# maniacs-oss/shadow

Measured on AMD Instinct MI355X. Metric: routing-table build GTEPS + packet-routes/sec at 1/2/4/8 MI355X (%HBM roofline), higher is better.
Workload: dtype f64

## Files before the change

### shadow_amd/csrc/topo_sssp_batch.hip

```cpp
#include <hip/hip_runtime.h>
#include <hipcub/hipcub.hpp>

#include <algorithm>
#include <cmath>
#include <cstddef>
#include <cstdint>
#include <type_traits>

#include "topo_dev_common.h"

namespace shdtopo {

namespace {

using namespace dev;

constexpr int kBatchRB = 2;
constexpr int kBatchU = 2;
constexpr int kBChunk = 512;
#ifndef SHD_BATCH_WRCOUNT
#define SHD_BATCH_WRCOUNT 0
#endif
#ifndef SHD_BATCH_TIME
#define SHD_BATCH_TIME 0
// ... 186 lines not shown
template <int K>
__device__ __forceinline__ double h0_bound(const LdsB<K>& L, const BView<K>& D, uint32_t j) {
    return fmin(L.hs[j], bits2d(D.get(0u, j)));
}

struct BBuckets {
    double inv_delta;
    uint32_t cb;
    uint32_t tie_tag;
};

constexpr uint32_t kTagMask = 0x3FFFFFFFu;
constexpr uint32_t kTagClaim = 0x40000000u;
static_assert(kTagMask == kPairTagMask && kTagClaim == kPairTagClaim, "the pair walks' tag (topo_device.h)");
constexpr uint32_t kTagTie = 0x80000000u;
__device__ __forceinline__ bool tag_claimed(uint32_t w, uint32_t ep) {
    return (w & ~kTagTie) == (ep | kTagClaim);
}
__device__ __forceinline__ bool tag_tied(uint32_t w, uint32_t ep) {
    return (w & kTagTie) && (w & kTagMask) == ep;
}

__device__ __forceinline__ uint32_t kappa_cut(const DevCSR& g, float4 ks0, float4 ks1, double T,
                                              uint32_t r0, uint32_t deg) {
    if ((double)ks0.x > T) return 0;
    if ((double)ks0.y > T) return 1;
    if ((double)ks0.z > T) return 3;
    if ((double)ks0.w > T) return 7;
    if (kKProbes > 4) {
        if ((double)ks1.x > T) return 15;
        if ((double)ks1.y > T) return 31;
        if ((double)ks1.z > T) return 63;
        if ((double)ks1.w > T) return 127;
    }
    uint32_t lo = kKProbes > 4 ? 128u : 8u, hi = deg;
    while (lo < hi) {
        const uint32_t mid = (lo + hi) >> 1;
        if ((double)g.kap[r0 + mid] > T) hi = mid; else lo = mid + 1;
    }
    return lo;
}

template <int K, bool CUT = false, bool DIR = false>
__device__ __forceinline__ uint32_t load_chunk(const uint32_t* Q, uint32_t cnt, const DevCSR& g,
                                               LdsB<K>& L, const BView<K>& D,
                                               typename MaskOps<K>::M* mcur,
                                               typename MaskOps<K>::M* hcur, bool stats = true,
                                               uint32_t spec_to = 0u) {
    using MO = MaskOps<K>;
    const uint32_t tid = threadIdx.x;
    const unsigned long long t0 = wall_clock64();
    uint32_t deg = 0;
    unsigned long long act = 0;
    if (tid < cnt) {
        const uint32_t v = Q[tid];
        uint32_t m;
        if (v < D.H) {
            m = MO::take(hcur, v);
            if (spec_to) {
                const uint32_t xw = D.xb[(v * K) >> 5] >> ((v * K) & 31);
                for (int jj = 0; jj < K; jj++) {
                    if (((m >> jj) & 1u) || ((xw >> jj) & 1u)) continue;
                    const unsigned long long d = D.hd[(size_t)v * K + jj];
                    if (d != kInfBits && bkt(bits2d(d), L.sh[jj], L.invd) <= spec_to) m |= 1u << jj;
                }
                if (m) atomicOr(&D.xb[(v * K) >> 5], m << ((v * K) & 31));
            }
        } else {
            wl_count(L, WL_MASK_ST, true, mcur + v);
            m = MO::take(mcur, v);
        }
        const uint32_t* rp = (CUT || !DIR) ? g.rowptr : g.rowptr_in;
        const uint32_t r0 = rp[v], r1 = rp[v + 1];
        deg = m ? r1 - r0 : 0u;
        if (CUT && deg) {
            const float4 ks0 = g.ksum[kKProbes / 4 * (size_t)v];
            const float4 ks1 = kKProbes > 4 ? g.ksum[kKProbes / 4 * (size_t)v + 1] : ks0;
            double dv[K];
            if (v < D.H) {
#pragma unroll
                for (int jj = 0; jj < K; jj++) dv[jj] = bits2d(D.hd[(size_t)v * K + jj]);
            } else {
                typedef unsigned long long u64x2 __attribute__((ext_vector_type(2)));
                const u64x2* p = reinterpret_cast<const u64x2*>(D.dist + (size_t)v * K);
#pragma unroll
                for (int h = 0; h < K / 2; h++) {
                    const u64x2 x = __builtin_nontemporal_load(p + h);
                    dv[2 * h] = bits2d(x.x);
                    dv[2 * h + 1] = bits2d(x.y);
                }
            }
            double T = -INFINITY;
#pragma unroll
            for (int jj = 0; jj < K; jj++) {
                if (!((m >> jj) & 1u)) continue;
                L.val[tid * K + jj] = dv[jj];
                const double h = h0_bound(L, D, (uint32_t)jj);
                const double t = (h - dv[jj]) + 1e-5 * (h + dv[jj] + g.piMax) + 1e-9;
                T = t > T ? t : T;
            }
            const uint32_t c = kappa_cut(g, ks0, ks1, T, r0, deg);
            deg = c < deg ? c : deg;
        }
        act = (unsigned long long)deg * (unsigned long long)__popc(m);
        L.rs[tid] = r0;
        L.vx[tid] = v;
        L.msk[tid] = m;
        if (stats && v < D.H && deg) {
            atomicAdd(&L.dg[0], (unsigned long long)deg);
            atomicAdd(&L.dg[1], act);
        }
    }
    uint32_t total;
    const uint32_t off = block_excl_scan<kSsspBlock>(deg, L.wave, &total);
    if (tid < cnt) L.off[tid] = off;
    if (tid == 0) L.off[cnt] = total;
    act = wave_sum_u64(act);
    if (stats && (tid & 63) == 0 && act) atomicAdd(&L.cnt[0], act);
    if (!CUT) {
        for (uint32_t i = tid; i < cnt * K; i += kSsspBlock) {
            const uint32_t vi = i / K, jj = i % K;
            if ((L.msk[vi] >> jj) & 1u) L.val[i] = bits2d(D.get(L.vx[vi], jj));
        }
    }
    if (tid < (uint32_t)K) L.dh0[tid] = h0_bound(L, D, tid);
    __syncthreads();
    if (stats && tid == 0) {
        L.cnt[2] += total;
        L.cnt[3] += wall_clock64() - t0;
    }
    return total;
}

__device__ __forceinline__ double rec_pi(uint32_t p) {
    if (kKapInRec) return (double)(float)__builtin_bit_cast(_Float16, (unsigned short)(p >> 16));
    return (double)__uint_as_float(p);
}
__device__ __forceinline__ float rec_kap0(uint32_t p) {
    return (float)__builtin_bit_cast(_Float16, (unsigned short)(p & 0xFFFFu));
}

__device__ __forceinline__ bool kappa_useful(float k0, double h, double d, double pimax) {
    return (double)k0 <= (h - d) + 1e-5 * (h + d + pimax) + 1e-9;
}

template <int K>
__device__ __forceinline__ int chunk_slot(const LdsB<K>& L, uint32_t cnt, uint32_t e) {
    int lo = 0, hi = (int)cnt - 1;
    while (lo < hi) {
        const int mid = (lo + hi + 1) >> 1;
        if (L.off[mid] <= e) lo = mid; else hi = mid - 1;
    }
    return lo;
}

__device__ __forceinline__ uint32_t wave_excl_scan(uint32_t x, uint32_t* total) {
    const uint32_t lane = threadIdx.x & 63;
    uint32_t v = x;
#pragma unroll
    for (int o = 1; o < 64; o <<= 1) {
        const uint32_t y = __shfl_up(v, o, 64);
        if (lane >= (uint32_t)o) v += y;
    }
    *total = __shfl(v, 63, 64);
    return v - x;
}

__device__ __forceinline__ uint32_t slice_slot(const uint32_t* off, uint32_t cnt, uint32_t e) {
    uint32_t lo = 0, hi = cnt - 1;
    while (lo < hi) {
        const uint32_t mid = (lo + hi + 1) >> 1;
        if (off[mid] <= e) lo = mid; else hi = mid - 1;
    }
    return lo;
}

constexpr uint32_t kBSub = kBChunk / (kSsspBlock / 64);
template <int K>
__device__ __forceinline__ uint32_t load_sub(uint32_t qv, uint32_t cnt, uint32_t wb,
                                             const DevCSR& g, LdsB<K>& L, const BView<K>& D,
                                             typename MaskOps<K>::M* mcur) {
    using MO = MaskOps<K>;
    const uint32_t lane = threadIdx.x & 63;
    uint32_t deg = 0;
    unsigned long long act = 0;
    if (lane < K) L.dh0[lane] = h0_bound(L, D, lane);
    if (lane < cnt) {
        const uint32_t v = qv;
        wl_count(L, WL_MASK_ST, true, mcur + v);
        const uint32_t m = MO::take(mcur, v);
        rl_count(L, RL_CHUNK, true, mcur + v);
        rl_count(L, RL_CHUNK, true, g.rowptr + v);
        rl_count(L, RL_CHUNK, true, g.ksum + kKProbes / 4 * (size_t)v);
        rl_count(L, RL_CHUNK, true, D.dist + (size_t)v * K);
        const uint32_t r0 = g.rowptr[v], r1 = g.rowptr[v + 1];
        const float4 ks0 = g.ksum[kKProbes / 4 * (size_t)v];
        const float4 ks1 = kKProbes > 4 ? g.ksum[kKProbes / 4 * (size_t)v + 1] : ks0;
        double dv[K];
        {
            typedef unsigned long long u64x2 __attribute__((ext_vector_type(2)));
            const u64x2* p = reinterpret_cast<const u64x2*>(D.dist + (size_t)v * K);
#pragma unroll
            for (int h = 0; h < K / 2; h++) {
                const u64x2 x = __builtin_nontemporal_load(p + h);
                dv[2 * h] = bits2d(x.x);
                dv[2 * h + 1] = bits2d(x.y);
            }
        }
        deg = m ? r1 - r0 : 0u;
        if (deg) {
            double T = -INFINITY;
#pragma unroll
            for (int jj = 0; jj < K; jj++) {
                if (!((m >> jj) & 1u)) continue;
                L.val[(wb + lane) * K + jj] = dv[jj];
                const double h = h0_bound(L, D, (uint32_t)jj);
                const double t = (h - dv[jj]) + 1e-5 * (h + dv[jj] + g.piMax) + 1e-9;
                T = t > T ? t : T;
            }
            const uint32_t c = kappa_cut(g, ks0, ks1, T, r0, deg);
            deg = c < deg ? c : deg;
        }
        act = (unsigned long long)deg * (unsigned long long)__popc(m);
        L.rs[wb + lane] = r0;
        L.vx[wb + lane] = v;
        L.msk[wb + lane] = m;
    }
    uint32_t total;
    const uint32_t off = wave_excl_scan(deg, &total);
    if (lane < cnt) L.off[wb + lane] = off;
    act = wave_sum_u64(act);
    if (lane == 0) {
        if (act) atomicAdd(&L.cnt[0], act);
        atomicAdd(&L.cnt[2], (unsigned long long)total);
    }
    asm volatile("s_waitcnt lgkmcnt(0)" ::: "memory");
    __builtin_amdgcn_wave_barrier();
    return total;
}

template <int K, int UA, bool WAVE = false>
__device__ __forceinline__ void relax_batch_t(const uint32_t* Q, uint32_t nq, const DevCSR& g,
                                              LdsB<K>& L, const BView<K>& D,
                                              typename MaskOps<K>::M* mcur,
                                              typename MaskOps<K>::M* hdef,
                                              typename MaskOps<K>::M* mnxt, uint32_t* qout,
                                              uint32_t qcap, uint32_t* hq, const BBuckets& B) {
    using MO = MaskOps<K>;
    static_assert(64 % K == 0, "a wave holds whole edge groups");
    static_assert(UA >= 1 && (UA & (UA - 1)) == 0, "the phase-B edge search halves UA * 64");
    constexpr int RB = kBatchRB;
    const uint32_t tid = threadIdx.x;
    const uint32_t lane = tid & 63;
    const uint32_t wv = tid >> 6;
    const uint32_t wb = WAVE ? wv * kBSub : 0u;
    uint32_t nb0 = 0, nqv = 0;
#if SHD_BATCH_TIME
    unsigned long long bt_last = wall_clock64();
#endif
    if (WAVE) {
        if (lane == 0) nb0 = atomicAdd(&L.qhead, kBSub);
        nb0 = __shfl(nb0, 0, 64);
        rl_count(L, RL_CHUNK, nb0 + lane < nq, Q + nb0 + lane);
        nqv = nb0 + lane < nq ? Q[nb0 + lane] : 0u;
    }
    for (uint32_t base = 0;; base += kBChunk) {
        uint32_t cnt, total;
        if (WAVE) {
            const uint32_t b0 = nb0, qv = nqv;
            if (b0 >= nq) break;
            cnt = min(kBSub, nq - b0);
            if (lane == 0) nb0 = atomicAdd(&L.qhead, kBSub);
            nb0 = __shfl(nb0, 0, 64);
            rl_count(L, RL_CHUNK, nb0 + lane < nq, Q + nb0 + lane);
            nqv = nb0 + lane < nq ? Q[nb0 + lane] : 0u;
            total = load_sub<K>(qv, cnt, wb, g, L, D, mcur);
        } else {
            if (base >= nq) break;
            cnt = min((uint32_t)kBChunk, nq - base);
            total = load_chunk<K, true>(Q + base, cnt, g, L, D, mcur, hdef, true,
                                        B.cb);
        }
        BT_TICK(0);
        constexpr uint32_t kStep = WAVE ? 64u : (uint32_t)kSsspBlock;
        for (uint32_t eb = 0; eb < total; eb += kStep * UA) {
            uint32_t an[UA], amk[UA], alo[UA], awl[UA], awh[UA], apb[UA];
#pragma unroll
            for (int a = 0; a < UA; a++) {
                const uint32_t e = eb + (uint32_t)a * kStep + (WAVE ? 0u : wv * 64) + lane;
                const bool valid = e < total;
                const int lo = !valid ? 0
                               : WAVE ? (int)(wb + slice_slot(L.off + wb, cnt, e))
                                      : chunk_slot<K>(L, cnt, e);
                const uint32_t jr = valid ? L.rs[lo] + (e - L.off[lo]) : 0u;
                rl_count(L, RL_PHASE_A, valid, g.adjk + kAdjWords * jr);
                const AdjRec r = *reinterpret_cast<const AdjRec*>(g.adjk + kAdjWords * jr);
                an[a] = r.a;
                apb[a] = r.p;
                awl[a] = r.b;
                awh[a] = r.c;
                amk[a] = valid ? L.msk[lo] : 0u;
                alo[a] = (uint32_t)lo;
            }
#pragma unroll
            for (int a = 0; a < UA; a++) {
                uint32_t mk = amk[a];
                const double w = __hiloint2double((int)awh[a], (int)awl[a]);
                const double pv = rec_pi(apb[a]);
                const bool skippable = kKapInRec && g.tflags &&
                                       (an[a] & 0x3FFFFFFFu) >= D.H && !((an[a] >> 30) & 1u);
                const float kz0 = rec_kap0(apb[a]);
                if (skippable && g.tflags == 2 && kz0 == INFINITY) {
                    mk = 0u;
                    amk[a] = 0u;
                }
                while (mk) {
                    const uint32_t jj = (uint32_t)__ffs(mk) - 1u;
                    mk &= mk - 1u;
                    const double ad = __dadd_rn(L.val[alo[a] * K + jj], w);
                    const double bnd = __dmul_rn(__dadd_rn(L.dh0[jj], pv), 1.000001);
                    if (ad > bnd || (skippable && !kappa_useful(kz0, L.dh0[jj], ad, g.piMax)))
                        amk[a] &= ~(1u << jj);
                }
            }
            uint32_t po[UA], ph[UA];
            uint32_t npt = 0, nph = 0;
#pragma unroll
            for (int a = 0; a < UA; a++) {
                const uint32_t c = (uint32_t)__popc(amk[a]);
                const bool tl = (an[a] & (g.tflags ? 0x3FFFFFFFu : 0x7FFFFFFFu)) >= D.H;
                uint32_t tt, th = 0;
                po[a] = npt + wave_excl_scan(tl ? c : 0u, &tt);
                ph[a] = nph + wave_excl_scan(tl ? 0u : c, &th);
                npt += tt;
                nph += th;
            }
            const uint32_t rT = (npt + 63u) / 64u;
            const uint32_t nround = rT + (nph + 63u) / 64u;
            uint32_t alm[UA];
#pragma unroll
            for (int a = 0; a < UA; a++) alm[a] = alo[a] | (amk[a] << 16);
            BT_TICK(1);
#if SHD_BATCH_TIME
            if (lane == 0) {
                atomicAdd(&L.bt[6], (unsigned long long)nround);
                atomicAdd(&L.bt[7], (unsigned long long)(npt + nph));
            }
#endif
            uint32_t fm = kNoBucket;
            for (uint32_t r0 = 0; r0 < nround; r0 += RB) {
            uint32_t n[RB], lo[RB], jr[RB], er[RB];
            unsigned long long ab[RB], cur[RB];
            float kz[RB];
            uint32_t tree[RB];
#pragma unroll
            for (int rr = 0; rr < RB; rr++) {
                const uint32_t r = r0 + (uint32_t)rr;
                const bool hubr = r >= rT;
                const uint32_t q = (hubr ? r - rT : r) * 64u + lane;
                const uint32_t lim = r >= nround ? 0u : hubr ? nph : npt;
                uint32_t pc[UA];
#pragma unroll
                for (int a = 0; a < UA; a++) pc[a] = hubr ? ph[a] : po[a];
                uint32_t e = 0;
#pragma unroll
                for (uint32_t st = (uint32_t)UA * 32u; st >= 1u; st >>= 1) {
                    const uint32_t c = e + st;
                    uint32_t oc = 0;
#pragma unroll
                    for (int a = 0; a < UA; a++) {
                        const uint32_t x = __shfl(pc[a], (int)(c & 63u), 64);
                        if ((c >> 6) == (uint32_t)a) oc = x;
                    }
                    if (oc <= q) e = c;
                }
                const int el = (int)(e & 63u);
                uint32_t xn = 0, xlm = 0, xwl = 0, xwh = 0, xpb = 0, xo = 0;
#pragma unroll
                for (int a = 0; a < UA; a++) {
                    const uint32_t t0 = __shfl(an[a], el, 64), t1 = __shfl(alm[a], el, 64);
                    const uint32_t t2 = __shfl(awl[a], el, 64), t3 = __shfl(awh[a], el, 64);
                    const uint32_t t4 = kKapInRec ? __shfl(apb[a], el, 64) : 0u;
                    const uint32_t t5 = __shfl(pc[a], el, 64);
                    if ((e >> 6) == (uint32_t)a) {
                        xn = t0; xlm = t1; xwl = t2; xwh = t3; xpb = t4; xo = t5;
                    }
                }
                bool on = q < lim;
                uint32_t mk = xlm >> 16, k = q - xo, jj = 0;
#pragma unroll
                for (uint32_t wdt = (uint32_t)K / 2u; wdt >= 1u; wdt >>= 1) {
                    const uint32_t c = (uint32_t)__popc(mk & ((1u << wdt) - 1u));
                    if (k >= c) { k -= c; jj += wdt; mk >>= wdt; }
                }
                jr[rr] = jj;
                n[rr] = xn & (g.tflags ? 0x3FFFFFFFu : 0x7FFFFFFFu);
                tree[rr] = xn >> 31;
                lo[rr] = xlm & 0xFFFFu;
                const double w = __hiloint2double((int)xwh, (int)xwl);
                const double abd = __dadd_rn(L.val[lo[rr] * K + jj], w);
                if (kKapInRec) kz[rr] = rec_kap0(xpb);
                er[rr] = on ? e : 0x10000u + lane;
                ab[rr] = on ? d2bits(abd) : ~0ull;
                const bool t = on && n[rr] >= D.H;
                rl_count(L, RL_RELAX_PRE, t, D.dist + (t ? (size_t)n[rr] : (size_t)0) * K + jj);
                const unsigned long long x = D.dist[(t ? (size_t)n[rr] : (size_t)0) * K + jj];
#if SHD_BATCH_TIME
                {
                    const unsigned long long tb = __ballot(t), hb = __ballot(on && !t);
                    if (lane == 0) {
                        if (tb) atomicAdd(&L.sw[0], 1ull);
                        atomicAdd(&L.sw[1], (unsigned long long)__popcll(tb));
                        atomicAdd(&L.sw[2], (unsigned long long)__popcll(hb));
                    }
                }
#endif
                if (!kKapInRec) kz[rr] = g.kap0[t ? n[rr] : 0u];
                cur[rr] = t ? x : 0ull;
            }
            unsigned long long old[RB];
            uint32_t pm[RB];
            bool hfv[RB];
#pragma unroll
            for (int rr = 0; rr < RB; rr++) {
                const bool on = ab[rr] != ~0ull;
                const uint32_t jj = jr[rr];
                const bool hub = n[rr] < D.H;
                bool nr = false, nf = false, ft = false;
                old[rr] = ~0ull;
                if (on && hub) {
                    const size_t wi = (size_t)n[rr] * K + jj;
                    const unsigned long long o = atomicMin(&D.hd[wi], ab[rr]);
                    const bool im = ab[rr] < o;
                    if (im) atomicAnd(&D.xb[wi >> 5], ~(1u << (wi & 31)));
                    if (n[rr] < D.P) {
                        wl_count(L, WL_HUB, im, D.hpar + wi);
                        if (im) D.hpar[wi] = L.vx[lo[rr]];
                        else if (ab[rr] == o) atomicOr(&D.tb[wi >> 5], 1u << (wi & 31));
                    }
                    if (im) {
                        const uint32_t b = bkt(bits2d(ab[rr]), L.sh[jj], B.inv_delta);
                        if (b <= B.cb) nr = true;
                        else fm = b < fm ? b : fm;
                    }
                } else if (on && ab[rr] <= cur[rr]) {
                    wl_count(L, WL_RELAX_MIN, true, &D.dist[(size_t)n[rr] * K + jj]);
                    old[rr] = atomicMin(&D.dist[(size_t)n[rr] * K + jj], ab[rr]);
                    if (ab[rr] < cur[rr]) {
                        const uint32_t b = bkt(bits2d(ab[rr]), L.sh[jj], B.inv_delta);
                        const bool inf = cur[rr] == kInfBits;
                        ft = inf;
                        if (b <= B.cb) nr = kappa_useful(kz[rr], L.dh0[jj], bits2d(ab[rr]), g.piMax);
                        else nf = inf;
                    }
                }
                uint32_t gm = nr ? 1u << jj : 0u, gf = (nf ? 1u : 0u) | (ft ? 2u : 0u);
#pragma unroll
                for (int o = 1; o < K; o <<= 1) {
                    const uint32_t ym = __shfl_down(gm, o, 64), yf = __shfl_down(gf, o, 64);
                    const uint32_t ye = __shfl_down(er[rr], o, 64);
                    if (lane + (uint32_t)o < 64u && ye == er[rr]) { gm |= ym; gf |= yf; }
                }
                const uint32_t pe = __shfl_up(er[rr], 1, 64);
                const bool head = on && (lane == 0 || pe != er[rr]);
                wl_count(L, WL_RELAX_TOUCH, head && gf, &D.pt[n[rr] >> 4]);
                wl_count(L, WL_RELAX_MASK, head && gm && !hub, mnxt + n[rr]);
                if (head && gf) (void)atomicOr(&D.pt[n[rr] >> 4], gf << (2u * (n[rr] & 15u)));
                pm[rr] = ~0u;
                hfv[rr] = false;
                if (head && gm) {
                    if (hub) hfv[rr] = MO::set(hdef, n[rr], gm) == 0u;
                    else pm[rr] = MO::set(mnxt, n[rr], gm);
                }
            }
#pragma unroll
            for (int rr = 0; rr < RB; rr++) {
                const uint32_t jj = jr[rr];
                if (old[rr] != ~0ull) {
                    const size_t wi = (size_t)n[rr] * K + jj;
                    const bool im = ab[rr] < old[rr];
                    wl_count(L, WL_RELAX_TIE, ab[rr] == old[rr], D.tpar + 4 * wi);
                    if (ab[rr] == old[rr]) D.tpar[4 * wi + 1] = B.tie_tag;
                    wl_count(L, WL_RELAX_HINT, im && !tree[rr], D.tpar + 4 * wi);
                    if (im && !tree[rr]) D.tpar[4 * wi] = L.vx[lo[rr]];
                    if (im) {
                        const uint32_t b = bkt(bits2d(ab[rr]), L.sh[jj], B.inv_delta);
                        if (b > B.cb) fm = b < fm ? b : fm;
                    }
                }
                wpush<K>(L, pm[rr] == 0u, n[rr], qout, &L.qtail, qcap, &L.fover, 1u);
                wpush<K>(L, hfv[rr], n[rr], hq, &L.htail, D.H, &L.fover, 1u);
            }
            }
            if (__ballot(fm != kNoBucket)) {
                fm = wave_min_u32(fm);
                if (lane == 0) atomicMin(&L.fminb, fm);
            }
            BT_TICK(2);
        }
        if (WAVE) {
            __builtin_amdgcn_wave_barrier();
            continue;
        }
        asm volatile("s_waitcnt vmcnt(0)" ::: "memory");
        __syncthreads();
    }
    if (WAVE) {
        asm volatile("s_waitcnt vmcnt(0)" ::: "memory");
        __syncthreads();
    }
}

template <int K, bool DIR, class VF, class EF>
__device__ __forceinline__ void expand_pairs(const uint32_t* Q, uint32_t nq, const DevCSR& g,
                                             LdsB<K>& L, VF&& vf, EF&& ef) {
    const uint32_t tid = threadIdx.x;
    for (uint32_t base = 0; base < nq; base += kBChunk) {
        const uint32_t cnt = min((uint32_t)kBChunk, nq - base);
        uint32_t deg = 0;
        if (tid < cnt) {
            const uint32_t q = Q[base + tid];
            double val = 0.0;
            vf(q, val);
            const uint32_t* rp = DIR ? g.rowptr_in : g.rowptr;
            const uint32_t r0 = rp[q / K], r1 = rp[q / K + 1];
            deg = r1 - r0;
            L.rs[tid] = r0;
            L.vx[tid] = q;
            L.val[tid] = val;
        }
        uint32_t total;
        const uint32_t off = block_excl_scan<kSsspBlock>(deg, L.wave, &total);
        if (tid < cnt) L.off[tid] = off;
        if (tid == 0) L.off[cnt] = total;
        __syncthreads();
        for (uint32_t e = tid; e < total; e += kSsspBlock) {
            const int lo = chunk_slot<K>(L, cnt, e);
            ef(L.vx[lo], L.val[lo], L.rs[lo] + (e - L.off[lo]));
        }
        __syncthreads();
    }
}

constexpr uint32_t kJobWalkSync = 1;
constexpr uint32_t kJobWalk = 2;
constexpr uint32_t kJobEpi = 3;
constexpr uint32_t kJobChunk = 256;
constexpr uint32_t kJobNone = 0xFFFFFFFFu;
constexpr uint32_t kNoPairS = 0xFFFFFFFFu;

}

template <int K, bool DIR, bool KEEP = false>
__global__ void __launch_bounds__(kSsspBlock, kBatchWgPerCu)
sssp_batch_kernel(DevCSR g, SlotWs ws, const uint32_t* __restrict__ sources,
                  const double* __restrict__ srcsh, const double* __restrict__ h0seed,
                  int nsrc, int kf,
                  const uint32_t* __restrict__ targets, int A, double delta, uint32_t H,
                  uint32_t P, uint32_t iter_guard,
                  double2* __restrict__ out_lr, uint16_t* __restrict__ out_hops,
                  double* __restrict__ out_rowmin, unsigned long long* __restrict__ stats) {
    using MO = MaskOps<K>;
    using M = typename MO::M;
    extern __shared__ __attribute__((aligned(16))) unsigned char smem[];
    LdsB<K>& L = *reinterpret_cast<LdsB<K>*>(smem);
    const BLayout lay = blayout<K>(H, P);
    M* hdef = reinterpret_cast<M*>(smem + lay.hdef);
    const uint32_t hmw = (uint32_t)((lay.tb - lay.hdef) / 4);
    const uint32_t tbw = (uint32_t)(((size_t)P * K + 31) / 32);
    const int slot = blockIdx.x;
    const uint32_t tid = threadIdx.x;
    const int64_t V = ws.V;
    BView<K> D;
    D.tb = reinterpret_cast<uint32_t*>(smem + lay.tb);
    D.xb = reinterpret_cast<uint32_t*>(smem + lay.xb);
    const uint32_t xbw = (uint32_t)(((size_t)H * K + 31) / 32);
    D.hd = reinterpret_cast<unsigned long long*>(smem + lay.hd);
    D.dist = ws.dist + (size_t)slot * (size_t)V * K;
    D.hpar = ws.hpar + (size_t)slot * (size_t)P * K;
    D.H = H;
    D.P = P;
    const size_t mbytes = ((size_t)V * sizeof(M) + 255) / 256 * 256;
    M* mA = reinterpret_cast<M*>(ws.mask + (size_t)slot * 2 * mbytes);
    M* mB = reinterpret_cast<M*>(ws.mask + (size_t)slot * 2 * mbytes + mbytes);
    uint32_t* qa = reinterpret_cast<uint32_t*>(ws.qa + (size_t)slot * ws.q_stride);
    uint32_t* qb = reinterpret_cast<uint32_t*>(ws.qb + (size_t)slot * ws.q_stride);
    uint4* prec = ws.prec + (size_t)slot * V * K;
    uint32_t* precw = reinterpret_cast<uint32_t*>(prec);
    D.tpar = precw;
    double* pbuf = ws.pathbuf + (size_t)slot * kPathBufPerSlot;
    uint32_t* ctr = ws.counters + (size_t)slot * 4;
    const uint32_t cap = (uint32_t)V;
    BBuckets B;
    B.inv_delta = 1.0 / delta;
    uint32_t* fscr = reinterpret_cast<uint32_t*>(ws.ring) + (size_t)slot * ws.ring_entries;
    uint32_t* vscr = fscr + (size_t)V * K;
    D.pt = reinterpret_cast<uint32_t*>((reinterpret_cast<uintptr_t>(vscr + (size_t)V) + 7) &
                                       ~(uintptr_t)7);
    const uint32_t pw = (uint32_t)((V + 31) / 32);
    unsigned long long* const pt2 = reinterpret_cast<unsigned long long*>(D.pt);
    constexpr unsigned long long kPendBits = 0x5555555555555555ull;
    const uint32_t pcap = (uint32_t)(V * K);

    uint32_t iter = ctr[0];
    if (tid < 4) L.cnt[tid] = 0;
    if (tid < 5) L.pt[tid] = 0;
    if (tid < 4) L.dg[tid] = 0;
    if (tid < 8) L.bt[tid] = 0;
    if (tid < 4) L.sw[tid] = 0;
    if (tid < 16) L.wl[tid] = 0;
    if (tid < 16) L.rl[tid] = 0;
    if (tid == 0) L.touched = 0;
    if (tid < 5) L.wk[tid] = 0;
    if (tid < 4) L.ev[tid] = 0;
    if (tid < 5) L.tm[tid] = 0;
    auto tick = [&](int i) {
        if (tid == 0) {
            const unsigned long long t = wall_clock64();
            L.tm[i] += t - L.tk;
            L.tk = t;
        }
    };

    if (tid == 0) {
        L.jcur = 0;
        L.fover = 0;
    }
    const uint32_t lane = tid & 63u;
    constexpr uint32_t kNoPair = 0xFFFFFFFFu;
    struct Hop {
        uint4 sp;
        double sl;
        unsigned long long d;
    };

    auto run_job = [&](uint32_t kind, uint32_t n, uint32_t epv, uint32_t r0v, uint32_t nkv,
                       uint32_t list) {
        unsigned long long* const distO = D.dist;
        uint4* const precO = prec;
        uint32_t* const precwO = precw;
        const uint32_t eptv = epv | kTagClaim;
        auto grab = [&](uint32_t* cnt) -> uint32_t {
            uint32_t b = kJobNone, c = 0;
            if (lane == 0) {
                const uint32_t x = atomicAdd(&L.jcur, kJobChunk);
                if (x < n) {
                    b = x;
                    c = min(kJobChunk, n - x);
                }
            }
            *cnt = __shfl(c, 0, 64);
            return __shfl(b, 0, 64);
        };
        if (kind != kJobEpi) {
            const uint32_t* P = list ? qb : qa;
            uint32_t* const S = fscr;
            const uint32_t pcapS = (uint32_t)(V * K);
            const bool gs = kind == kJobWalkSync;
            auto put = [&](uint32_t q, uint32_t u, double loss) {
                const unsigned long long lb = d2bits(loss);
                wl_count(L, WL_PREC, true, precO + q);
                precO[q] = make_uint4(u, eptv, (uint32_t)lb, (uint32_t)(lb >> 32));
            };
            auto load_hop = [&](uint32_t v, uint32_t j) -> Hop {
                Hop hh;
                const uint32_t q = v * K + j;
                rl_count(L, RL_WALK, v >= H, reinterpret_cast<const uint4*>(g.spt) + 2 * (size_t)v);
                rl_count(L, RL_WALK, true, distO + (size_t)q);
                if (v >= H) {
                    const uint4* sp = reinterpret_cast<const uint4*>(g.spt) + 2 * (size_t)v;
                    hh.sp = sp[0];
                    const uint2 l = *reinterpret_cast<const uint2*>(sp + 1);
                    hh.sl = __hiloint2double((int)l.y, (int)l.x);
                } else {
                    hh.sp = make_uint4(0xFFFFFFFFu, 0u, 0u, 0u);
                    hh.sl = 0.0;
                }
                hh.d = ld_l2_u64(&distO[(size_t)q]);
                return hh;
            };
            uint32_t i = 0, iend = 0, q = 0, j = 0;
            uint32_t nw = 0, nw0 = 0;
            bool act = false, fresh = false, more = true;
            Hop h;
            h.sp = make_uint4(0xFFFFFFFFu, 0u, 0u, 0u);
            h.sl = 0.0;
            h.d = 0ull;
            for (;;) {
                if (more && !__any(i < iend)) {
                    uint32_t c;
                    const uint32_t b = grab(&c);
                    if (b == kJobNone) {
                        more = false;
                    } else {
                        i = b + lane;
                        iend = b + c;
                    }
                }
                bool take = !act && i < iend;
                if (gs) {
                    const unsigned long long am = __ballot(act);
                    take = take && ((am >> (lane & ~(uint32_t)(K - 1))) & ((1ull << K) - 1ull)) == 0ull;
                }
                rl_count(L, RL_WALK, take, P + (take ? i : 0u));
                if (take) {
                    q = P[i];
                    i += 64;
                    j = q % K;
                    act = q != kNoPair;
                    fresh = act;
                }
                if (!more && !__any(act || i < iend)) break;
                bool sp = false;
                if (act && fresh) {
                    h = load_hop(q / K, j);
                    fresh = false;
                } else if (act) {
                    const uint32_t v = q / K;
                    const uint32_t pu = h.sp.x;
                    const bool tree = v >= H && pu < (uint32_t)V;
                    Hop hn = h;
                    if (tree) hn = load_hop(pu, j);
                    rl_count(L, RL_WALK, true, precwO + 4 * (size_t)q);
                    const uint32_t tw = ld_l2_u32(&precwO[4 * (size_t)q + 1]);
                    if (tag_claimed(tw, epv)) {
                        act = false;
                    } else {
                        nw++;
                        const bool tied = tag_tied(tw, epv);
                        if (tree && !tied &&
                            __dadd_rn(bits2d(hn.d), __hiloint2double((int)h.sp.w, (int)h.sp.z)) ==
                                bits2d(h.d)) {
                            put(q, pu, h.sl);
                            nw0++;
                            if (pu == L.src[j]) {
                                act = false;
                            } else {
                                q = pu * K + j;
                                h = hn;
                            }
                        } else {
                            wl_count(L, WL_PREC, true, precwO + 4 * (size_t)q);
                            precwO[4 * (size_t)q + 1] = eptv | (tied ? kTagTie : 0u);
                            sp = true;
                            act = false;
                        }
                    }
                }
                const unsigned long long m = __ballot(sp);
                if (m) {
                    const uint32_t need = (uint32_t)__popcll(m);
                    uint32_t x = 0;
                    if (lane == 0) x = atomicAdd(&L.qtail, need);
                    const uint32_t base = __shfl(x, 0, 64);
                    if (sp) {
                        const uint32_t pos = base + (uint32_t)__popcll(m & ((1ull << lane) - 1ull));
                        wl_count(L, WL_QUEUE, pos < pcapS, S + pos);
                        if (pos < pcapS) S[pos] = q;
                        else atomicOr(&L.fover, 128u);
                    }
                }
            }
            const unsigned long long s0 = wave_sum_u64(nw), s1 = wave_sum_u64(nw0);
            if (lane == 0) {
                atomicAdd(&L.wk[0], s0);
                atomicAdd(&L.wk[1], s1);
            }
        } else {
            double* lpb = reinterpret_cast<double*>(smem + lay.hd);
            const uint32_t nl = H * K / kSsspBlock;
            auto pb_at = [&](uint32_t x) -> double* {
                return x < nl ? lpb + (size_t)x * kSsspBlock + tid : pbuf + (size_t)x * kSsspBlock + tid;
            };
            unsigned long long* const rminP = L.rmin;
            for (;;) {
                uint32_t c;
                const uint32_t b = grab(&c);
                if (b == kJobNone) break;
                for (uint32_t i = b + lane; i < b + c; i += 64) {
                    const uint32_t jj = i % nkv;
                    const uint32_t k = i / nkv;
                    uint32_t t, lu = kNoLeaf;
                    double lw = 0.0, ll = 0.0;
                    if (ws.tleaf) {
                        rl_count(L, RL_EPI, true, ws.tleaf + 2 * (size_t)k);
                        const uint4 la = ws.tleaf[2 * (size_t)k];
                        const uint2 lb = *reinterpret_cast<const uint2*>(ws.tleaf + 2 * (size_t)k + 1);
                        t = la.x;
                        lu = la.y;
                        lw = __hiloint2double((int)la.w, (int)la.z);
                        ll = __hiloint2double((int)lb.y, (int)lb.x);
                    } else {
                        rl_count(L, RL_EPI, true, targets + k);
                        t = targets[k];
// ... 1478 lines not shown
```

Baseline: 2582.

## Relax hub-destination edges inline during filtering, skipping redistribution rounds

Hub-vertex edge relaxations move out of the compacted round-based redistribution loop and run directly in the per-edge filter loop. A plain read-before-atomic check skips atomicMin when the candidate cannot improve the hub distance. Hub edges then no longer use scan slots, shuffles or rounds, which removes the separate hub prefix scan. In exchange, hub work runs lane-divergent inside a serial per-lane mask loop, and the per-target mask merging across lanes for hub vertices is lost, so hdef sets and pushes happen per lane rather than per wave-merged group.

Result: no change. 2591, median of 2 (+0.3%).

```diff
diff --git a/shadow_amd/csrc/topo_sssp_batch.hip b/shadow_amd/csrc/topo_sssp_batch.hip
--- a/shadow_amd/csrc/topo_sssp_batch.hip
+++ b/shadow_amd/csrc/topo_sssp_batch.hip
@@ -512,11 +512,17 @@
                 amk[a] = valid ? L.msk[lo] : 0u;
                 alo[a] = (uint32_t)lo;
             }
+            uint32_t fm = kNoBucket;
+#if SHD_BATCH_TIME
+            uint32_t hseen = 0, hdrop = 0;
+#endif
 #pragma unroll
             for (int a = 0; a < UA; a++) {
                 uint32_t mk = amk[a];
                 const double w = __hiloint2double((int)awh[a], (int)awl[a]);
                 const double pv = rec_pi(apb[a]);
+                const uint32_t nn = an[a] & (g.tflags ? 0x3FFFFFFFu : 0x7FFFFFFFu);
+                const bool hub = nn < D.H;
                 const bool skippable = kKapInRec && g.tflags &&
                                        (an[a] & 0x3FFFFFFFu) >= D.H && !((an[a] >> 30) & 1u);
                 const float kz0 = rec_kap0(apb[a]);
@@ -524,29 +530,62 @@
                     mk = 0u;
                     amk[a] = 0u;
                 }
+                uint32_t gm = 0u;
                 while (mk) {
                     const uint32_t jj = (uint32_t)__ffs(mk) - 1u;
                     mk &= mk - 1u;
                     const double ad = __dadd_rn(L.val[alo[a] * K + jj], w);
                     const double bnd = __dmul_rn(__dadd_rn(L.dh0[jj], pv), 1.000001);
-                    if (ad > bnd || (skippable && !kappa_useful(kz0, L.dh0[jj], ad, g.piMax)))
+                    if (ad > bnd || (skippable && !kappa_useful(kz0, L.dh0[jj], ad, g.piMax))) {
                         amk[a] &= ~(1u << jj);
-                }
-            }
-            uint32_t po[UA], ph[UA];
-            uint32_t npt = 0, nph = 0;
+                        continue;
+                    }
+                    if (!hub) continue;
+                    const size_t wi = (size_t)nn * K + jj;
+                    const unsigned long long ab = d2bits(ad);
+                    const bool noeff = ab > D.hd[wi];
+#if SHD_BATCH_TIME
+                    hseen++;
+                    hdrop += noeff ? 1u : 0u;
+#endif
+                    if (noeff) continue;
+                    const unsigned long long o = atomicMin(&D.hd[wi], ab);
+                    const bool im = ab < o;
+                    if (im) atomicAnd(&D.xb[wi >> 5], ~(1u << (wi & 31)));
+                    if (nn < D.P) {
+                        wl_count(L, WL_HUB, im, D.hpar + wi);
+                        if (im) D.hpar[wi] = L.vx[alo[a]];
+                        else if (ab == o) atomicOr(&D.tb[wi >> 5], 1u << (wi & 31));
+                    }
+                    if (im) {
+                        const uint32_t b = bkt(ad, L.sh[jj], B.inv_delta);
+                        if (b <= B.cb) gm |= 1u << jj;
+                        else fm = b < fm ? b : fm;
+                    }
+                }
+                if (hub) amk[a] = 0u;
+                const bool hfv = gm && MO::set(hdef, nn, gm) == 0u;
+                wpush<K>(L, hfv, nn, hq, &L.htail, D.H, &L.fover, 1u);
+            }
+#if SHD_BATCH_TIME
+            {
+                const unsigned long long hs = wave_sum_u64((unsigned long long)hseen);
+                const unsigned long long hp = wave_sum_u64((unsigned long long)hdrop);
+                if (lane == 0 && hs) {
+                    atomicAdd(&L.sw[2], hs);
+                    atomicAdd(&L.sw[3], hp);
+                }
+            }
+#endif
+            uint32_t po[UA];
+            uint32_t npt = 0;
 #pragma unroll
             for (int a = 0; a < UA; a++) {
-                const uint32_t c = (uint32_t)__popc(amk[a]);
-                const bool tl = (an[a] & (g.tflags ? 0x3FFFFFFFu : 0x7FFFFFFFu)) >= D.H;
-                uint32_t tt, th = 0;
-                po[a] = npt + wave_excl_scan(tl ? c : 0u, &tt);
-                ph[a] = nph + wave_excl_scan(tl ? 0u : c, &th);
+                uint32_t tt;
+                po[a] = npt + wave_excl_scan((uint32_t)__popc(amk[a]), &tt);
                 npt += tt;
-                nph += th;
-            }
-            const uint32_t rT = (npt + 63u) / 64u;
-            const uint32_t nround = rT + (nph + 63u) / 64u;
+            }
+            const uint32_t nround = (npt + 63u) / 64u;
             uint32_t alm[UA];
 #pragma unroll
             for (int a = 0; a < UA; a++) alm[a] = alo[a] | (amk[a] << 16);
@@ -554,10 +593,9 @@
 #if SHD_BATCH_TIME
             if (lane == 0) {
                 atomicAdd(&L.bt[6], (unsigned long long)nround);
-                atomicAdd(&L.bt[7], (unsigned long long)(npt + nph));
+                atomicAdd(&L.bt[7], (unsigned long long)npt);
             }
 #endif
-            uint32_t fm = kNoBucket;
             for (uint32_t r0 = 0; r0 < nround; r0 += RB) {
             uint32_t n[RB], lo[RB], jr[RB], er[RB];
             unsigned long long ab[RB], cur[RB];
@@ -566,12 +604,7 @@
 #pragma unroll
             for (int rr = 0; rr < RB; rr++) {
                 const uint32_t r = r0 + (uint32_t)rr;
-                const bool hubr = r >= rT;
-                const uint32_t q = (hubr ? r - rT : r) * 64u + lane;
-                const uint32_t lim = r >= nround ? 0u : hubr ? nph : npt;
-                uint32_t pc[UA];
-#pragma unroll
-                for (int a = 0; a < UA; a++) pc[a] = hubr ? ph[a] : po[a];
+                const uint32_t q = r * 64u + lane;
                 uint32_t e = 0;
 #pragma unroll
                 for (uint32_t st = (uint32_t)UA * 32u; st >= 1u; st >>= 1) {
@@ -579,7 +612,7 @@
                     uint32_t oc = 0;
 #pragma unroll
                     for (int a = 0; a < UA; a++) {
-                        const uint32_t x = __shfl(pc[a], (int)(c & 63u), 64);
+                        const uint32_t x = __shfl(po[a], (int)(c & 63u), 64);
                         if ((c >> 6) == (uint32_t)a) oc = x;
                     }
                     if (oc <= q) e = c;
@@ -591,12 +624,12 @@
                     const uint32_t t0 = __shfl(an[a], el, 64), t1 = __shfl(alm[a], el, 64);
                     const uint32_t t2 = __shfl(awl[a], el, 64), t3 = __shfl(awh[a], el, 64);
                     const uint32_t t4 = kKapInRec ? __shfl(apb[a], el, 64) : 0u;
-                    const uint32_t t5 = __shfl(pc[a], el, 64);
+                    const uint32_t t5 = __shfl(po[a], el, 64);
                     if ((e >> 6) == (uint32_t)a) {
                         xn = t0; xlm = t1; xwl = t2; xwh = t3; xpb = t4; xo = t5;
                     }
                 }
-                bool on = q < lim;
+                const bool on = q < npt;
                 uint32_t mk = xlm >> 16, k = q - xo, jj = 0;
 #pragma unroll
                 for (uint32_t wdt = (uint32_t)K / 2u; wdt >= 1u; wdt >>= 1) {
@@ -612,16 +645,15 @@
                 if (kKapInRec) kz[rr] = rec_kap0(xpb);
                 er[rr] = on ? e : 0x10000u + lane;
                 ab[rr] = on ? d2bits(abd) : ~0ull;
-                const bool t = on && n[rr] >= D.H;
+                const bool t = on;
                 rl_count(L, RL_RELAX_PRE, t, D.dist + (t ? (size_t)n[rr] : (size_t)0) * K + jj);
                 const unsigned long long x = D.dist[(t ? (size_t)n[rr] : (size_t)0) * K + jj];
 #if SHD_BATCH_TIME
                 {
-                    const unsigned long long tb = __ballot(t), hb = __ballot(on && !t);
+                    const unsigned long long tb = __ballot(t);
                     if (lane == 0) {
                         if (tb) atomicAdd(&L.sw[0], 1ull);
                         atomicAdd(&L.sw[1], (unsigned long long)__popcll(tb));
-                        atomicAdd(&L.sw[2], (unsigned long long)__popcll(hb));
                     }
                 }
 #endif
@@ -630,30 +662,13 @@
             }
             unsigned long long old[RB];
             uint32_t pm[RB];
-            bool hfv[RB];
 #pragma unroll
             for (int rr = 0; rr < RB; rr++) {
                 const bool on = ab[rr] != ~0ull;
                 const uint32_t jj = jr[rr];
-                const bool hub = n[rr] < D.H;
                 bool nr = false, nf = false, ft = false;
                 old[rr] = ~0ull;
-                if (on && hub) {
-                    const size_t wi = (size_t)n[rr] * K + jj;
-                    const unsigned long long o = atomicMin(&D.hd[wi], ab[rr]);
-                    const bool im = ab[rr] < o;
-                    if (im) atomicAnd(&D.xb[wi >> 5], ~(1u << (wi & 31)));
-                    if (n[rr] < D.P) {
-                        wl_count(L, WL_HUB, im, D.hpar + wi);
-                        if (im) D.hpar[wi] = L.vx[lo[rr]];
-                        else if (ab[rr] == o) atomicOr(&D.tb[wi >> 5], 1u << (wi & 31));
-                    }
-                    if (im) {
-                        const uint32_t b = bkt(bits2d(ab[rr]), L.sh[jj], B.inv_delta);
-                        if (b <= B.cb) nr = true;
-                        else fm = b < fm ? b : fm;
-                    }
-                } else if (on && ab[rr] <= cur[rr]) {
+                if (on && ab[rr] <= cur[rr]) {
                     wl_count(L, WL_RELAX_MIN, true, &D.dist[(size_t)n[rr] * K + jj]);
                     old[rr] = atomicMin(&D.dist[(size_t)n[rr] * K + jj], ab[rr]);
                     if (ab[rr] < cur[rr]) {
@@ -674,14 +689,10 @@
                 const uint32_t pe = __shfl_up(er[rr], 1, 64);
                 const bool head = on && (lane == 0 || pe != er[rr]);
                 wl_count(L, WL_RELAX_TOUCH, head && gf, &D.pt[n[rr] >> 4]);
-                wl_count(L, WL_RELAX_MASK, head && gm && !hub, mnxt + n[rr]);
+                wl_count(L, WL_RELAX_MASK, head && gm, mnxt + n[rr]);
                 if (head && gf) (void)atomicOr(&D.pt[n[rr] >> 4], gf << (2u * (n[rr] & 15u)));
                 pm[rr] = ~0u;
-                hfv[rr] = false;
-                if (head && gm) {
-                    if (hub) hfv[rr] = MO::set(hdef, n[rr], gm) == 0u;
-                    else pm[rr] = MO::set(mnxt, n[rr], gm);
-                }
+                if (head && gm) pm[rr] = MO::set(mnxt, n[rr], gm);
             }
 #pragma unroll
             for (int rr = 0; rr < RB; rr++) {
@@ -699,7 +710,6 @@
                     }
                 }
                 wpush<K>(L, pm[rr] == 0u, n[rr], qout, &L.qtail, qcap, &L.fover, 1u);
-                wpush<K>(L, hfv[rr], n[rr], hq, &L.htail, D.H, &L.fover, 1u);
             }
             }
             if (__ballot(fm != kNoBucket)) {
```
